# lucaspk512/vrdone

Hardware: AMD Instinct MI355X
Metric: subject-object pairs/sec forward (2048 pairs x 256 frames x 512-d) (higher is better)
Workload: dtype f16x3: f32 products as 3 scaled-f16 MFMA products (~22-bit), f32 accumulate; reference-grade: distance to a float64 run of the reference <= 1.4 x the reference's own float32 error (tests/golden/mask_vrd_f64.npz)

## Files before the change

vrdone_amd/csrc/vrd_rowops.hip:

```cpp
#include "vrd_common.h"
#include "vrd_box_feats.h"
#include <cmath>

namespace {

constexpr float LN_EPS = 1e-5f;

__device__ __forceinline__ float4 ld4(const float* p) { return *reinterpret_cast<const float4*>(p); }
__device__ __forceinline__ void st4(float* p, float4 v) { *reinterpret_cast<float4*>(p) = v; }
__device__ __forceinline__ float4 f4add(float4 a, float4 b) { return make_float4(a.x + b.x, a.y + b.y, a.z + b.z, a.w + b.w); }

__global__ __launch_bounds__(256) void bct_to_btc_kernel(const float* __restrict__ src, int C_total, int T, int c0,
                                                         int count, float* __restrict__ dst, int64_t ld_dst, int pair, int T_src,
                                                         const int32_t* __restrict__ src_batch, unsigned* rflag) {
    __shared__ float tile[64][65];
    vrd::RangeTrack rt;
    const int b = blockIdx.z, ct = blockIdx.y * 64, tt = blockIdx.x * 64;
    const int tx = threadIdx.x & 63, ty = threadIdx.x >> 6;
    const float* s = src + ((int64_t)(src_batch ? src_batch[b] : b) * C_total + c0) * T_src;
    for (int c = ty; c < 64; c += 4)
        tile[c][tx] = (ct + c < count && tt + tx < T) ? s[(int64_t)(ct + c) * T_src + tt + tx] : 0.f;
    __syncthreads();
    for (int t = ty; t < 64; t += 4)
        if (tt + t < T && ct + tx < count) {
            float* row = dst + ((int64_t)b * T + tt + t) * ld_dst;
            if (pair) vrd::store_pair1(row, ct + tx, count, tile[tx][t], pair, &rt);
            else row[ct + tx] = tile[tx][t];
        }
    rt.report(rflag, vrd::RANGE_INPUT);
}

__global__ __launch_bounds__(256) void bct_to_btc_vec_kernel(const float* __restrict__ src, int C_total, int T, int c0,
                                                             int count, float* __restrict__ dst, int64_t ld_dst, int pair, int T_src,
                                                             const int32_t* __restrict__ src_batch, unsigned* rflag) {
    __shared__ float tile[64][65];
    vrd::RangeTrack rt;
    const int b = blockIdx.z, ct = blockIdx.y * 64, tt = blockIdx.x * 64;
    const float* s = src + ((int64_t)(src_batch ? src_batch[b] : b) * C_total + c0) * T_src;
    {
        const int tx = threadIdx.x & 15, ty = threadIdx.x >> 4;
#pragma unroll
        for (int c = ty; c < 64; c += 16) {
            float4 v = make_float4(0.f, 0.f, 0.f, 0.f);
            if (ct + c < count && tt + 4 * tx < T) v = ld4(s + (int64_t)(ct + c) * T_src + tt + 4 * tx);
            tile[c][4 * tx] = v.x, tile[c][4 * tx + 1] = v.y, tile[c][4 * tx + 2] = v.z, tile[c][4 * tx + 3] = v.w;
        }
    }
    __syncthreads();
#pragma unroll
    for (int k = 0; k < 4; ++k) {
        const int id = threadIdx.x + 256 * k;
        const int cg = id & 15, t = id >> 4;
        if (tt + t >= T || ct + 4 * cg >= count) continue;
        const float4 v = make_float4(tile[4 * cg][t], tile[4 * cg + 1][t], tile[4 * cg + 2][t], tile[4 * cg + 3][t]);
        float* row = dst + ((int64_t)b * T + tt + t) * ld_dst;
        if (pair) vrd::store_pair4(row, ct + 4 * cg, count, v, pair, &rt);
        else st4(row + ct + 4 * cg, v);
    }
    rt.report(rflag, vrd::RANGE_INPUT);
}

__global__ __launch_bounds__(256) void btc_to_bct_kernel(const float* __restrict__ src, int64_t ld_src, int C, int T,
                                                         float* __restrict__ dst) {
    __shared__ float tile[64][65];
    const int b = blockIdx.z, ct = blockIdx.y * 64, tt = blockIdx.x * 64;
    const int tx = threadIdx.x & 63, ty = threadIdx.x >> 6;
    for (int t = ty; t < 64; t += 4)
        tile[t][tx] = (tt + t < T && ct + tx < C) ? src[((int64_t)b * T + tt + t) * ld_src + ct + tx] : 0.f;
    __syncthreads();
    for (int c = ty; c < 64; c += 4)
        if (ct + c < C && tt + tx < T) dst[((int64_t)b * C + ct + c) * T + tt + tx] = tile[tx][c];
}

__device__ __forceinline__ void pack_segment(const float* src, bool live, int lane, int width, float* dst, int pair,
                                             vrd::RangeTrack* rt = nullptr) {
    for (int c = lane; c < width; c += 64) {
        const float v = live ? src[c] : 0.f;
        if (pair) vrd::store_pair1(dst, c, width, v, pair, rt);
        else dst[c] = v;
    }
}

__global__ __launch_bounds__(256) void pack_pairs_kernel(vrd_pack_args a, unsigned* rflag) {
    vrd::RangeTrack rt;
    const int lane = threadIdx.x & 63;
    const int64_t row = (int64_t)blockIdx.x * 4 + __builtin_amdgcn_readfirstlane(threadIdx.x >> 6);
    if (row >= (int64_t)a.P * a.T) return;
    const int p = (int)(row / a.T), t = (int)(row - (int64_t)p * a.T);
    const bool live = t < a.lens[p];
    const float* src = a.src[p] + (int64_t)t * a.C_in;
    const int64_t half = (int64_t)a.P * a.T;
    int c0 = 0;
    pack_segment(src + c0, live, lane, a.V, a.vis + row * a.V, a.pair_wide, &rt);              c0 += a.V;
    pack_segment(src + c0, live, lane, a.V, a.vis + (half + row) * a.V, a.pair_wide, &rt);     c0 += a.V;
    if (a.Cc) {
        pack_segment(src + c0, live, lane, a.Cc, a.clip + row * a.Cc, a.pair_wide, &rt);          c0 += a.Cc;
        pack_segment(src + c0, live, lane, a.Cc, a.clip + (half + row) * a.Cc, a.pair_wide, &rt); c0 += a.Cc;
    }
    pack_segment(src + c0, live, lane, a.S, a.so_box + row * a.S, 0);                     c0 += a.S;
    pack_segment(src + c0, live, lane, a.E, a.ent + row * a.E, 0);                        c0 += a.E;
    pack_segment(src + c0, live, lane, a.E, a.ent + (half + row) * a.E, 0);
    rt.report(rflag, vrd::RANGE_INPUT);
}

using vrd::Box4;
using vrd::load_box;
using vrd::entity_feats;

__global__ __launch_bounds__(256) void gather_pairs_kernel(vrd_gather_args a, unsigned* rflag) {
    vrd::RangeTrack rt;
    const int lane = threadIdx.x & 63;
    const int64_t row = (int64_t)blockIdx.x * 4 + __builtin_amdgcn_readfirstlane(threadIdx.x >> 6);
    if (row >= (int64_t)a.P * a.T) return;
    const int p = (int)(row / a.T), t = (int)(row - (int64_t)p * a.T);
    const int n = a.lens[p];
    const bool live = t < n;
    const int64_t rs = a.s_row[p] + (int64_t)t * a.stride, ro = a.o_row[p] + (int64_t)t * a.stride;
    const int64_t half = (int64_t)a.P * a.T;
    if (a.out_vis) {
        pack_segment(a.vis + (live ? rs : 0) * a.V, live, lane, a.V, a.out_vis + row * a.V, a.pair_wide, &rt);
        pack_segment(a.vis + (live ? ro : 0) * a.V, live, lane, a.V, a.out_vis + (half + row) * a.V, a.pair_wide, &rt);
        if (a.Cc) {
            pack_segment(a.clip + (live ? rs : 0) * a.Cc, live, lane, a.Cc, a.out_clip + row * a.Cc, a.pair_wide, &rt);
            pack_segment(a.clip + (live ? ro : 0) * a.Cc, live, lane, a.Cc, a.out_clip + (half + row) * a.Cc, a.pair_wide, &rt);
        }
        rt.report(rflag, vrd::RANGE_INPUT);
    }
    float* const so = a.out_so_box + row * 5;
    float* const es = a.out_ent + row * 8;
    float* const eo = a.out_ent + (half + row) * 8;
    if (!live) {
        if (lane < 5) so[lane] = 0.f;
        if (lane < 8) es[lane] = 0.f, eo[lane] = 0.f;
        return;
    }
    if (lane == 0) {
        float f[5];
        vrd::so_box_feats(load_box(a.boxes, rs), load_box(a.boxes, ro), f);
#pragma unroll
        for (int i = 0; i < 5; ++i) so[i] = f[i];
    } else if (lane == 1 || lane == 2) {
        float f[8];
        const float w = a.seq_wh ? a.seq_wh[2 * (int64_t)p] : a.w, h = a.seq_wh ? a.seq_wh[2 * (int64_t)p + 1] : a.h;
        entity_feats(a.boxes, lane == 1 ? a.s_row[p] : a.o_row[p], a.stride, t, n, w, h, f);
        float* const dst = lane == 1 ? es : eo;
#pragma unroll
        for (int i = 0; i < 8; ++i) dst[i] = f[i];
    }
}

__global__ __launch_bounds__(256) void assemble_pairs_kernel(vrd_assemble_args a) {
    const int lane = threadIdx.x & 63;
    const int64_t row = (int64_t)blockIdx.x * 4 + __builtin_amdgcn_readfirstlane(threadIdx.x >> 6);
    if (row >= 2 * (int64_t)a.P * a.T) return;
    const int e = (int)(row / a.T), t = (int)(row - (int64_t)e * a.T);
    const int side = e >= a.P, p = e - side * a.P;
    const int n = a.lens[p];
    const float* src = nullptr;
    if (t < n) {
        const int64_t piece = ((int64_t)side * 2 * a.P + p) * a.L;
        const int end_len = n == a.T ? a.L : a.piece;
        if (n <= a.piece || t < a.reach) src = a.snippets + (piece + t) * a.D;
        else if (t >= n - a.reach) src = a.snippets + (piece + (int64_t)a.P * a.L + (t - (n - end_len))) * a.D;
        else src = a.streams + (a.stream_row[e] + t) * a.D;
    }
    float4* dst = reinterpret_cast<float4*>(a.out + row * a.D);
    for (int c = lane; c < a.D / 4; c += 64) dst[c] = src ? reinterpret_cast<const float4*>(src)[c] : float4{0.f, 0.f, 0.f, 0.f};
}

template <int NV, bool WIDE>
__device__ __forceinline__ int lane_chan(int i, int lane) { return WIDE ? lane * 8 + i * 4 : i * 256 + lane * 4; }

template <int NV, bool WIDE = false>
__device__ __forceinline__ void ln_rows(float4 (&v)[NV], const float* gamma, const float* beta, int lane, bool relu) {
    constexpr float inv_c = 1.0f / (256.0f * NV);
    float s = 0.f;
#pragma unroll
    for (int i = 0; i < NV; ++i) s += (v[i].x + v[i].y) + (v[i].z + v[i].w);
    const float mean = vrd::wave_sum(s) * inv_c;
    float ss = 0.f;
#pragma unroll
    for (int i = 0; i < NV; ++i) {
        v[i].x -= mean; v[i].y -= mean; v[i].z -= mean; v[i].w -= mean;
        ss += (v[i].x * v[i].x + v[i].y * v[i].y) + (v[i].z * v[i].z + v[i].w * v[i].w);
    }
    const float inv = 1.0f / sqrtf(vrd::wave_sum(ss) * inv_c + LN_EPS);
#pragma unroll
    for (int i = 0; i < NV; ++i) {
        const float4 g = ld4(gamma + lane_chan<NV, WIDE>(i, lane)), bb = ld4(beta + lane_chan<NV, WIDE>(i, lane));
        v[i].x = fmaf(v[i].x * inv, g.x, bb.x);
        v[i].y = fmaf(v[i].y * inv, g.y, bb.y);
        v[i].z = fmaf(v[i].z * inv, g.z, bb.z);
        v[i].w = fmaf(v[i].w * inv, g.w, bb.w);
        if (relu) {
            v[i].x = fmaxf(v[i].x, 0.f); v[i].y = fmaxf(v[i].y, 0.f);
            v[i].z = fmaxf(v[i].z, 0.f); v[i].w = fmaxf(v[i].w, 0.f);
        }
    }
}

template <int NV>
__global__ __launch_bounds__(256) void layernorm_kernel(const float* __restrict__ x, int64_t ldx, float* __restrict__ y,
                                                        int64_t ldy, int64_t rows, const float* __restrict__ gamma,
                                                        const float* __restrict__ beta, int relu,
                                                        const float* __restrict__ post_add, int64_t ld_add, int period,
                                                        int pair, unsigned* rflag) {
    vrd::RangeTrack rt;
    const int lane = threadIdx.x & 63;
    int64_t row = (int64_t)blockIdx.x * 4 + __builtin_amdgcn_readfirstlane(threadIdx.x >> 6);
    const int64_t stride = (int64_t)gridDim.x * 4;
    if (row >= rows) return;
    float4 v[NV], vn[NV];
#pragma unroll
    for (int i = 0; i < NV; ++i) v[i] = ld4(x + row * ldx + i * 256 + lane * 4);
    for (;;) {
        const int64_t nxt = row + stride;
        if (nxt < rows) {
#pragma unroll
            for (int i = 0; i < NV; ++i) vn[i] = ld4(x + nxt * ldx + i * 256 + lane * 4);
        }
        ln_rows<NV>(v, gamma, beta, lane, relu != 0);
        if (post_add) {
            const float* a = post_add + (row % period) * ld_add;
#pragma unroll
            for (int i = 0; i < NV; ++i) v[i] = f4add(v[i], ld4(a + i * 256 + lane * 4));
        }
#pragma unroll
        for (int i = 0; i < NV; ++i) {
            if (pair) vrd::store_pair4(y + row * ldy, i * 256 + lane * 4, 256 * NV, v[i], pair, &rt);
            else st4(y + row * ldy + i * 256 + lane * 4, v[i]);
        }
        if (nxt >= rows) break;
        row = nxt;
#pragma unroll
        for (int i = 0; i < NV; ++i) v[i] = vn[i];
    }
    rt.report(rflag, vrd::RANGE_LAYERNORM);
}

constexpr int CL_MAXK = 32;
template <int NV>
__global__ __launch_bounds__(256) void conv_ln_kernel(vrd_conv_ln_args p, unsigned* rflag) {
    vrd::RangeTrack rt;
    constexpr int N = 256 * NV;
    constexpr bool WIDE = NV == 2;
    extern __shared__ __attribute__((aligned(16))) float cl_lds[];
    const int K = p.Cin * p.taps;
    for (int idx = threadIdx.x; idx < N * K; idx += 256) {
        const int n = idx / K, rem = idx - n * K, ci = rem / p.taps, tap = rem - ci * p.taps;
        cl_lds[(tap * p.Cin + ci) * N + n] = p.w[idx];
    }
    for (int n = threadIdx.x; n < N; n += 256) cl_lds[K * N + n] = p.bias ? p.bias[n] : 0.f;
    __syncthreads();
    const int lane = threadIdx.x & 63;
    constexpr int RG = 4;
    int64_t grp = (int64_t)blockIdx.x * 4 + __builtin_amdgcn_readfirstlane(threadIdx.x >> 6);
    const int64_t stride = (int64_t)gridDim.x * 4;
    const int half = p.taps / 2;
    const int lrow = lane / p.Cin, lci = lane - lrow * p.Cin;
    auto load_in = [&](int64_t g) {
        const int64_t r = g * RG - half + lrow;
        float val = 0.f;
        if (lrow < RG + 2 * half && r >= 0 && r < p.rows) val = p.x[r * p.ldx + lci];
        return val;
    };
    float xin = grp * RG < p.rows ? load_in(grp) : 0.f;
    for (; grp * RG < p.rows; grp += stride) {
        const int64_t row0 = grp * RG;
        const float xcur = xin;
        if ((grp + stride) * RG < p.rows) xin = load_in(grp + stride);
        float4 v[RG][NV];
        int t[RG];
#pragma unroll
        for (int j = 0; j < RG; ++j) {
            t[j] = (int)((row0 + j) % p.T);
#pragma unroll
            for (int i = 0; i < NV; ++i) v[j][i] = *reinterpret_cast<const float4*>(cl_lds + K * N + lane_chan<NV, WIDE>(i, lane));
        }
        for (int tap = 0; tap < p.taps; ++tap) {
            for (int ci = 0; ci < p.Cin; ++ci) {
                const float* wk = cl_lds + (tap * p.Cin + ci) * N;
                float4 w[NV];
#pragma unroll
                for (int i = 0; i < NV; ++i) w[i] = *reinterpret_cast<const float4*>(wk + lane_chan<NV, WIDE>(i, lane));
#pragma unroll
                for (int j = 0; j < RG; ++j) {
                    const int tt = t[j] + tap - half;
                    const bool ok = tt >= 0 && tt < p.T && row0 + j < p.rows;
                    const float xl = __builtin_bit_cast(float, __builtin_amdgcn_readlane(__builtin_bit_cast(int, xcur), (j + tap) * p.Cin + ci));
                    const float xv = ok ? xl : 0.f;
#pragma unroll
                    for (int i = 0; i < NV; ++i) {
                        v[j][i].x = fmaf(w[i].x, xv, v[j][i].x); v[j][i].y = fmaf(w[i].y, xv, v[j][i].y);
                        v[j][i].z = fmaf(w[i].z, xv, v[j][i].z); v[j][i].w = fmaf(w[i].w, xv, v[j][i].w);
                    }
                }
            }
        }
#pragma unroll
        for (int j = 0; j < RG; ++j) {
            const int64_t row = row0 + j;
            if (row >= p.rows) break;
            if (p.row_mask) {
                const float mk = (float)vrd::uniform_load(p.row_mask + row);
#pragma unroll
                for (int i = 0; i < NV; ++i) v[j][i].x *= mk, v[j][i].y *= mk, v[j][i].z *= mk, v[j][i].w *= mk;
            }
            if (p.gamma) {
                ln_rows<NV, WIDE>(v[j], p.gamma, p.beta, lane, p.relu != 0);
            } else if (p.relu) {
#pragma unroll
                for (int i = 0; i < NV; ++i) {
                    v[j][i].x = fmaxf(v[j][i].x, 0.f); v[j][i].y = fmaxf(v[j][i].y, 0.f);
                    v[j][i].z = fmaxf(v[j][i].z, 0.f); v[j][i].w = fmaxf(v[j][i].w, 0.f);
                }
            }
            float* yr = p.y + row * p.ldy;
            if (WIDE && p.out_pair) {
                vrd::store_pair8(yr, lane * 8, v[j][0], v[j][NV - 1], p.out_pair, &rt);
            } else {
#pragma unroll
                for (int i = 0; i < NV; ++i) {
                    const int c = lane_chan<NV, WIDE>(i, lane);
                    if (p.out_pair) vrd::store_pair4(yr, c, N, v[j][i], p.out_pair, &rt);
                    else st4(yr + c, v[j][i]);
                }
            }
        }
    }
    rt.report(rflag, vrd::RANGE_LAYERNORM);
}

constexpr int DW_RW = 16;

template <int NV, int KS, int GIN>
__global__ __launch_bounds__(256) void dwconv_ln_kernel(vrd_dwconv_ln_args p, int Tout_u, int strips_per_seq, int strips_per_wave, int rw, unsigned* rflag,
                                                        vrd::SegTable sg) {
    vrd::RangeTrack rt;
    constexpr int C = 256 * NV, NT = GIN * KS, SETF = (NT + 3) * C;
    constexpr bool WIDE = NV == 2 && GIN == 1;
    extern __shared__ __attribute__((aligned(16))) float dw_lds[];
    const int lane = threadIdx.x & 63, wave = __builtin_amdgcn_readfirstlane(threadIdx.x >> 6);
    for (int o = 0; o < p.n_out; ++o) {
        float* const ls = dw_lds + o * SETF;
        if (p.packed[o]) {
            for (int idx = threadIdx.x * 4; idx < SETF; idx += 1024) st4(ls + idx, ld4(p.packed[o] + idx));
            continue;
        }
        for (int idx = threadIdx.x; idx < C * NT; idx += 256) ls[(idx % NT) * C + idx / NT] = p.w[o][idx];
        for (int c = threadIdx.x; c < C; c += 256) {
            ls[NT * C + c] = p.bias[o] ? p.bias[o][c] : 0.f;
            ls[(NT + 1) * C + c] = p.gamma[o] ? p.gamma[o][c] : 1.f;
            ls[(NT + 2) * C + c] = p.gamma[o] ? p.beta[o][c] : 0.f;
        }
    }
    const float* const pre = dw_lds + p.n_out * SETF;
    if (p.pre_gamma)
        for (int c = threadIdx.x; c < C; c += 256) {
            dw_lds[p.n_out * SETF + c] = p.pre_gamma[c];
            dw_lds[p.n_out * SETF + C + c] = p.pre_beta[c];
        }
    __syncthreads();
    const int nwg = gridDim.x, bid = blockIdx.x;
    const int xcd = bid & 7, qq = nwg >> 3, rem = nwg & 7;
    const int lid = (xcd < rem ? xcd * (qq + 1) : rem * (qq + 1) + (xcd - rem) * qq) + (bid >> 3);
    for (int si = 0; si < strips_per_wave; ++si) {
    const int64_t ws = ((int64_t)lid * 4 + wave) * strips_per_wave + si;
    int Tin, Tout, to0;
    int64_t xrow0, urow0, orow0;
    if (sg.count) {
        int g, b, strip;
        if (!vrd::seg_find(sg, ws, g, b, strip)) break;
        Tin = sg.T[g], Tout = Tin / p.stride, to0 = strip * rw;
        xrow0 = sg.row[g] + (int64_t)b * Tin;
        urow0 = sg.row[g] / 2 + (int64_t)b * (Tin / 2);
        orow0 = sg.row[g] / p.stride + (int64_t)b * Tout;
    } else {
        const int b = (int)(ws / strips_per_seq);
        if (b >= p.B) break;
        Tin = p.Tin, Tout = Tout_u, to0 = (int)(ws - (int64_t)b * strips_per_seq) * rw;
        xrow0 = (int64_t)b * Tin, urow0 = (int64_t)b * (Tin / 2), orow0 = (int64_t)b * Tout;
    }
    const int to1 = min(to0 + rw, Tout);

    struct Row {
        float4 v[NV][GIN];
    };
    auto load_row = [&](int ti) {
        Row r;
        const bool ok = ti >= 0 && ti < Tin;
#pragma unroll
        for (int i = 0; i < NV; ++i)
#pragma unroll
            for (int g = 0; g < GIN; ++g) {
                float4 v = make_float4(0.f, 0.f, 0.f, 0.f);
                if (ok) {
                    const int64_t coff = (int64_t)GIN * lane_chan<NV, WIDE>(i, lane) + 4 * g;
                    v = ld4(p.x + (xrow0 + ti) * p.ldx + coff);
                    if (p.x_up) v = f4add(v, ld4(p.x_up + (urow0 + (ti >> 1)) * p.ldx_up + coff));
                }
                r.v[i][g] = v;
            }
        if (GIN == 1 && p.pre_gamma && ok) {
            float4 t[NV];
#pragma unroll
            for (int i = 0; i < NV; ++i) t[i] = r.v[i][0];
            ln_rows<NV, WIDE>(t, pre, pre + C, lane, false);
#pragma unroll
            for (int i = 0; i < NV; ++i) r.v[i][0] = t[i];
        }
        return r;
    };
    if (p.mask_out) {
        const int64_t r0 = orow0 + to0;
        const bool mine = lane < to1 - to0 && p.mask_out[r0 + lane] != 0;
        if (!__any(mine)) {
#pragma unroll
            for (int o = 0; o < 3; ++o) {
                if (o >= p.n_out) break;
                const float* const lb = dw_lds + o * SETF + (NT + 2) * C;
                float4 val[NV];
#pragma unroll
                for (int i = 0; i < NV; ++i) {
                    val[i] = *reinterpret_cast<const float4*>(lb + lane_chan<NV, WIDE>(i, lane));
                    if (p.relu[o]) {
                        val[i].x = fmaxf(val[i].x, 0.f); val[i].y = fmaxf(val[i].y, 0.f);
                        val[i].z = fmaxf(val[i].z, 0.f); val[i].w = fmaxf(val[i].w, 0.f);
                    }
                }
                for (int to = to0; to < to1; ++to) {
                    const int64_t row = orow0 + to;
                    if (WIDE && p.out_pair[o]) {
                        vrd::store_pair8(p.y[o] + row * p.ldy[o], lane * 8, val[0], val[NV - 1], p.out_pair[o], &rt);
                    } else {
#pragma unroll
                        for (int i = 0; i < NV; ++i) {
                            const int c = lane_chan<NV, WIDE>(i, lane);
                            if (p.out_pair[o]) vrd::store_pair4(p.y[o] + row * p.ldy[o], c, 256 * NV, val[i], p.out_pair[o], &rt);
                            else st4(p.y[o] + row * p.ldy[o] + c, val[i]);
                        }
                    }
                }
            }
            continue;
        }
    }
    Row win[KS];
#pragma unroll
    for (int k = 0; k < KS; ++k) win[k] = load_row(p.stride * to0 + k - KS / 2);
    for (int to = to0; to < to1; ++to) {
        Row nxt[2];
        const int tn = p.stride * (to + 1) - KS / 2;
        const bool more = to + 1 < to1;
        if (KS == 1) {
            if (more) nxt[0] = load_row(tn);
        } else if (p.stride == 1) {
            if (more) nxt[0] = load_row(tn + 2);
        } else {
            if (more) {
                nxt[0] = load_row(tn + 1);
                nxt[1] = load_row(tn + 2);
            }
        }
        const int64_t row = orow0 + to;
        const float mk = p.mask_out ? (float)p.mask_out[row] : 1.f;
#pragma unroll
        for (int o = 0; o < 3; ++o) {
            if (o >= p.n_out) break;
            const float* const ls = dw_lds + o * SETF;
            float4 acc[NV];
#pragma unroll
            for (int i = 0; i < NV; ++i) {
                const int c = lane_chan<NV, WIDE>(i, lane);
                float4 r = *reinterpret_cast<const float4*>(ls + NT * C + c);
#pragma unroll
                for (int k = 0; k < KS; ++k) {
                    if (GIN == 1) {
                        const float4 w = *reinterpret_cast<const float4*>(ls + k * C + c);
                        const float4 v = win[k].v[i][0];
                        r.x += w.x * v.x; r.y += w.y * v.y; r.z += w.z * v.z; r.w += w.w * v.w;
                    } else {
                        const float4 w0 = *reinterpret_cast<const float4*>(ls + (0 * KS + k) * C + c);
                        const float4 w1 = *reinterpret_cast<const float4*>(ls + (1 * KS + k) * C + c);
                        const float4 v0 = win[k].v[i][0], v1 = win[k].v[i][GIN - 1];
                        r.x += w0.x * v0.x + w1.x * v0.y;
                        r.y += w0.y * v0.z + w1.y * v0.w;
                        r.z += w0.z * v1.x + w1.z * v1.y;
                        r.w += w0.w * v1.z + w1.w * v1.w;
                    }
                }
                acc[i] = make_float4(r.x * mk, r.y * mk, r.z * mk, r.w * mk);
            }
            if (p.gamma[o]) {
                ln_rows<NV, WIDE>(acc, ls + (NT + 1) * C, ls + (NT + 2) * C, lane, p.relu[o] != 0);
            } else if (p.relu[o]) {
#pragma unroll
                for (int i = 0; i < NV; ++i) {
                    acc[i].x = fmaxf(acc[i].x, 0.f); acc[i].y = fmaxf(acc[i].y, 0.f);
                    acc[i].z = fmaxf(acc[i].z, 0.f); acc[i].w = fmaxf(acc[i].w, 0.f);
                }
            }
            if (WIDE && p.out_pair[o]) {
                vrd::store_pair8(p.y[o] + row * p.ldy[o], lane * 8, acc[0], acc[NV - 1], p.out_pair[o], &rt);
            } else {
#pragma unroll
                for (int i = 0; i < NV; ++i) {
                    const int c = lane_chan<NV, WIDE>(i, lane);
                    if (p.out_pair[o]) vrd::store_pair4(p.y[o] + row * p.ldy[o], c, 256 * NV, acc[i], p.out_pair[o], &rt);
                    else st4(p.y[o] + row * p.ldy[o] + c, acc[i]);
                }
            }
        }
        if (more) {
            if (KS == 1) {
                win[0] = nxt[0];
            } else if (p.stride == 1) {
                win[0] = win[1];
                win[KS > 1 ? 1 : 0] = win[KS - 1];
                win[KS - 1] = nxt[0];
            } else {
                win[0] = win[KS - 1];
                win[KS > 1 ? 1 : 0] = nxt[0];
                win[KS - 1] = nxt[1];
            }
        }
    }
    }
    rt.report(rflag, vrd::RANGE_DWCONV_LN);
}

__global__ __launch_bounds__(256) void maxpool_mask_kernel(const float* __restrict__ x, int64_t ldx, int B, int Tin, int C,
                                                           const uint8_t* __restrict__ mask_in, float* __restrict__ y,
                                                           int64_t ldy, uint8_t* __restrict__ mask_out) {
    const int c4 = C / 4;
    const int64_t idx = (int64_t)blockIdx.x * 256 + threadIdx.x;
    const int Tout = Tin / 2;
    if (idx >= (int64_t)B * Tout * c4) return;
    const int c = (int)(idx % c4) * 4;
    const int64_t row = idx / c4;
    const int b = (int)(row / Tout), to = (int)(row - (int64_t)b * Tout);
    const float* base = x + ((int64_t)b * Tin + 2 * to) * ldx + c;
    float4 m = ld4(base);
    const float4 r = ld4(base + ldx);
    m.x = fmaxf(m.x, r.x); m.y = fmaxf(m.y, r.y); m.z = fmaxf(m.z, r.z); m.w = fmaxf(m.w, r.w);
    if (to > 0) {
        const float4 l = ld4(base - ldx);
        m.x = fmaxf(m.x, l.x); m.y = fmaxf(m.y, l.y); m.z = fmaxf(m.z, l.z); m.w = fmaxf(m.w, l.w);
    }
    const uint8_t mk = mask_in[(int64_t)b * Tin + 2 * to];
    const float f = (float)mk;
    st4(y + row * ldy + c, make_float4(m.x * f, m.y * f, m.z * f, m.w * f));
    if (c == 0 && mask_out) mask_out[row] = mk;
}

constexpr int MH_D = 256, MH_TT = 32, MH_QMAX = 16;

__global__ __launch_bounds__(256) void mask_head_kernel(const float* __restrict__ emb, int64_t ld_emb,
                                                        const float* __restrict__ feat, int64_t ld_feat,
                                                        const uint8_t* __restrict__ out_mask, int Q, int T, float fill,
                                                        float* __restrict__ seg) {
    __shared__ float fs[MH_TT][MH_D + 1];
    __shared__ float es[MH_QMAX][MH_D];
    const int b = blockIdx.y, t0 = blockIdx.x * MH_TT, tid = threadIdx.x;
    for (int i = tid; i < MH_TT * (MH_D / 4); i += 256) {
        const int r = i / (MH_D / 4), c = (i % (MH_D / 4)) * 4;
        float4 v = make_float4(0.f, 0.f, 0.f, 0.f);
        if (t0 + r < T) v = ld4(feat + ((int64_t)b * T + t0 + r) * ld_feat + c);
        fs[r][c] = v.x; fs[r][c + 1] = v.y; fs[r][c + 2] = v.z; fs[r][c + 3] = v.w;
    }
    for (int i = tid; i < Q * (MH_D / 4); i += 256) {
        const int r = i / (MH_D / 4), c = (i % (MH_D / 4)) * 4;
        st4(&es[r][c], ld4(emb + ((int64_t)b * Q + r) * ld_emb + c));
    }
    __syncthreads();
    const int tt = tid & 31, qg = tid >> 5;
    if (t0 + tt >= T) return;
    const bool on = out_mask[(int64_t)b * T + t0 + tt] != 0;
    for (int q = qg; q < Q; q += 8) {
        float s = 0.f;
#pragma unroll 8
        for (int c = 0; c < MH_D; ++c) s = fmaf(es[q][c], fs[tt][c], s);
        seg[((int64_t)b * Q + q) * T + t0 + tt] = on ? s : fill;
    }
}

inline bool aligned16(const void* ptr) { return (reinterpret_cast<uintptr_t>(ptr) & 15u) == 0; }

constexpr int RB_THREADS = 1024;
__global__ __launch_bounds__(RB_THREADS) void row_blocks_kernel(const uint8_t* __restrict__ mask, int nblocks, int seg_len, int S,
                                                                int32_t* __restrict__ order, int32_t* __restrict__ n_active) {
    __shared__ int counts[RB_THREADS];
    const int tid = threadIdx.x;
    const int per = (nblocks + RB_THREADS - 1) / RB_THREADS;
    const int b0 = min(tid * per, nblocks), b1 = min(b0 + per, nblocks);
    auto active = [&](int b) {
        const uint4* q = reinterpret_cast<const uint4*>(mask + (int64_t)b * 32);
        const uint4 lo = q[0], hi = q[1];
        return ((lo.x | lo.y | lo.z | lo.w | hi.x | hi.y | hi.z | hi.w) != 0u) ? 1 : 0;
    };
    int mine = 0;
    for (int b = b0; b < b1; ++b) mine += active(b);
    counts[tid] = mine;
    __syncthreads();
    for (int d = 1; d < RB_THREADS; d <<= 1) {
        const int v = tid >= d ? counts[tid - d] : 0;
        __syncthreads();
        counts[tid] += v;
        __syncthreads();
    }
    const int total = counts[RB_THREADS - 1];
    auto start = [&](int s) { return min(s * seg_len, nblocks); };
    auto first = [&](int s) { return (int)(((int64_t)total * start(s)) / nblocks); };
    auto pads_before = [&](int s) { return start(s) - first(s); };
    int a = counts[tid] - mine;
    int i = b0 - a;
    int sa = 0, sp = 0;
    for (int b = b0; b < b1; ++b) {
        if (active(b)) {
            while (sa + 1 < S && first(sa + 1) <= a) ++sa;
            order[start(sa) + (a - first(sa))] = b;
            ++a;
        } else {
            while (sp + 1 < S && pads_before(sp + 1) <= i) ++sp;
            order[start(sp) + (first(sp + 1) - first(sp)) + (i - pads_before(sp))] = b;
            ++i;
        }
    }
    if (tid < S) n_active[tid] = first(tid + 1) - first(tid);
}

}

extern "C" {

int vrd_bct_to_btc(const float* src, int B, int C_total, int T, int c0, int count, float* dst, int64_t ld_dst,
                   int out_pair, int T_src, const int32_t* src_batch, void* stream) {
    VRD_CHECK_ARG(src && dst, "vrd_bct_to_btc: null pointer");
    if (T_src == 0) T_src = T;
    VRD_CHECK_ARG(T_src >= T, "vrd_bct_to_btc: T_src (%d) < T (%d)", T_src, T);
    VRD_CHECK_ARG(B > 0 && T > 0 && count > 0 && c0 >= 0 && c0 + count <= C_total && ld_dst >= count,
                  "vrd_bct_to_btc: bad slab c0=%d count=%d C=%d ld=%lld", c0, count, C_total, (long long)ld_dst);
    VRD_CHECK_ARG(B <= 65535, "vrd_bct_to_btc: B too large for one launch (%d)", B);
    hipStream_t s = static_cast<hipStream_t>(stream);
    vrd::ProfScope prof(VRD_K_TRANSPOSE, s, 0.0, 8.0 * B * (double)count * T);
    dim3 grid((T + 63) / 64, (count + 63) / 64, B);
    VRD_CHECK_ARG(!out_pair || (count % 32 == 0 && ld_dst % 4 == 0 && aligned16(dst)), "vrd_bct_to_btc: pair rows need count %% 32 == 0");
    const bool vec = T % 4 == 0 && T_src % 4 == 0 && count % 4 == 0 && ld_dst % 4 == 0 && aligned16(dst) && aligned16(src);
    if (vec) hipLaunchKernelGGL(bct_to_btc_vec_kernel, grid, dim3(256), 0, s, src, C_total, T, c0, count, dst, ld_dst, out_pair, T_src, src_batch, out_pair == VRD_PAIR_F16 ? vrd::range_flag() : nullptr);
    else hipLaunchKernelGGL(bct_to_btc_kernel, grid, dim3(256), 0, s, src, C_total, T, c0, count, dst, ld_dst, out_pair, T_src, src_batch, out_pair == VRD_PAIR_F16 ? vrd::range_flag() : nullptr);
    VRD_LAUNCH_CHECK();
    return 0;
}

int vrd_pack_pairs(const vrd_pack_args* a, void* stream) {
    VRD_CHECK_ARG(a && a->src && a->lens && a->vis && a->so_box && a->ent, "vrd_pack_pairs: null pointer");
    VRD_CHECK_ARG(a->P > 0 && a->T > 0 && a->V > 0 && a->S > 0 && a->E > 0 && a->Cc >= 0, "vrd_pack_pairs: bad sizes");
    VRD_CHECK_ARG(a->C_in == 2 * a->V + 2 * a->Cc + a->S + 2 * a->E, "vrd_pack_pairs: C_in %d does not match the slab widths", a->C_in);
    VRD_CHECK_ARG(a->Cc == 0 || a->clip, "vrd_pack_pairs: clip buffer missing");
    VRD_CHECK_ARG(!a->pair_wide || (a->V % 32 == 0 && a->Cc % 32 == 0), "vrd_pack_pairs: pair rows need widths %% 32 == 0");
    hipStream_t s = static_cast<hipStream_t>(stream);
    const int64_t rows = (int64_t)a->P * a->T;
    vrd::ProfScope prof(VRD_K_TRANSPOSE, s, 0.0, 8.0 * (double)rows * a->C_in);
    hipLaunchKernelGGL(pack_pairs_kernel, dim3((unsigned)((rows + 3) / 4)), dim3(256), 0, s, *a, a->pair_wide == VRD_PAIR_F16 ? vrd::range_flag() : nullptr);
    VRD_LAUNCH_CHECK();
    return 0;
}

int vrd_gather_pairs(const vrd_gather_args* a, void* stream) {
    VRD_CHECK_ARG(a && a->vis && a->boxes && a->s_row && a->o_row && a->lens && a->out_so_box && a->out_ent,
                  "vrd_gather_pairs: null pointer");
    VRD_CHECK_ARG(a->P > 0 && a->T > 0 && a->V > 0 && a->Cc >= 0 && a->stride >= 1 && a->w > 0.f && a->h > 0.f, "vrd_gather_pairs: bad sizes");
    VRD_CHECK_ARG(a->Cc == 0 || !a->out_vis || (a->clip && a->out_clip), "vrd_gather_pairs: clip buffers missing");
    VRD_CHECK_ARG(!a->pair_wide || (a->V % 32 == 0 && a->Cc % 32 == 0), "vrd_gather_pairs: pair rows need widths %% 32 == 0");
    VRD_CHECK_ARG(aligned16(a->boxes), "vrd_gather_pairs: boxes must be 16-byte aligned");
    hipStream_t s = static_cast<hipStream_t>(stream);
    const int64_t rows = (int64_t)a->P * a->T;
    vrd::ProfScope prof(VRD_K_TRANSPOSE, s, 0.0, 8.0 * (double)rows * ((a->out_vis ? 2 * a->V + 2 * a->Cc : 0) + 21));
    hipLaunchKernelGGL(gather_pairs_kernel, dim3((unsigned)((rows + 3) / 4)), dim3(256), 0, s, *a, a->pair_wide == VRD_PAIR_F16 ? vrd::range_flag() : nullptr);
    VRD_LAUNCH_CHECK();
    return 0;
}

int vrd_assemble_pairs(const vrd_assemble_args* a, void* stream) {
    VRD_CHECK_ARG(a && a->streams && a->snippets && a->stream_row && a->lens && a->out, "vrd_assemble_pairs: null pointer");
    VRD_CHECK_ARG(a->P > 0 && a->T > 0 && a->D > 0 && a->D % 4 == 0, "vrd_assemble_pairs: bad sizes");
    VRD_CHECK_ARG(a->reach >= 0 && a->piece >= 2 * a->reach && a->piece >= 1 && a->L > a->piece && a->T >= a->L,
                  "vrd_assemble_pairs: pieces of %d frames in buffers of %d (T = %d) cannot cover a reach of %d", a->piece, a->L, a->T, a->reach);
    VRD_CHECK_ARG(aligned16(a->streams) && aligned16(a->snippets) && aligned16(a->out), "vrd_assemble_pairs: rows must be 16-byte aligned");
    hipStream_t s = static_cast<hipStream_t>(stream);
    const int64_t rows = 2 * (int64_t)a->P * a->T;
    VRD_CHECK_ARG((rows + 3) / 4 < ((int64_t)1 << 31), "vrd_assemble_pairs: grid too large");
    vrd::ProfScope prof(VRD_K_TRANSPOSE, s, 0.0, 8.0 * (double)rows * a->D);
    hipLaunchKernelGGL(assemble_pairs_kernel, dim3((unsigned)((rows + 3) / 4)), dim3(256), 0, s, *a);
    VRD_LAUNCH_CHECK();
    return 0;
}

int vrd_row_blocks(const uint8_t* mask, int64_t rows, int seg_len, int32_t* order, int32_t* n_active, void* stream) {
    VRD_CHECK_ARG(mask && order && n_active, "vrd_row_blocks: null pointer");
    VRD_CHECK_ARG(rows > 0 && rows % 32 == 0 && rows / 32 < (1 << 30), "vrd_row_blocks: rows %lld must be a positive multiple of 32", (long long)rows);
    const int nblocks = (int)(rows / 32);
    VRD_CHECK_ARG(seg_len >= 1 && (nblocks + seg_len - 1) / seg_len <= 64, "vrd_row_blocks: segment length %d gives more than 64 segments", seg_len);
    VRD_CHECK_ARG(aligned16(mask), "vrd_row_blocks: mask must be 16-byte aligned");
    hipStream_t s = static_cast<hipStream_t>(stream);
    vrd::ProfScope prof(VRD_K_TRANSPOSE, s, 0.0, (double)rows + 4.0 * nblocks);
    hipLaunchKernelGGL(row_blocks_kernel, dim3(1), dim3(RB_THREADS), 0, s, mask, nblocks, seg_len, (nblocks + seg_len - 1) / seg_len, order, n_active);
    VRD_LAUNCH_CHECK();
    return 0;
}

int vrd_btc_to_bct(const float* src, int64_t ld_src, int B, int C, int T, float* dst, void* stream) {
    VRD_CHECK_ARG(src && dst, "vrd_btc_to_bct: null pointer");
    VRD_CHECK_ARG(B > 0 && B <= 65535 && T > 0 && C > 0 && ld_src >= C, "vrd_btc_to_bct: bad shape");
    hipStream_t s = static_cast<hipStream_t>(stream);
    vrd::ProfScope prof(VRD_K_TRANSPOSE, s, 0.0, 8.0 * B * (double)C * T);
    dim3 grid((T + 63) / 64, (C + 63) / 64, B);
    hipLaunchKernelGGL(btc_to_bct_kernel, grid, dim3(256), 0, s, src, ld_src, C, T, dst);
    VRD_LAUNCH_CHECK();
    return 0;
}

int vrd_layernorm(const float* x, int64_t ldx, float* y, int64_t ldy, int64_t rows, int C, const float* gamma,
                  const float* beta, int relu, const float* post_add, int64_t ld_add, int add_period, int out_pair,
                  void* stream) {
    VRD_CHECK_ARG(x && y && gamma && beta, "vrd_layernorm: null pointer");
    VRD_CHECK_ARG(C == 256 || C == 512, "vrd_layernorm: C must be 256 or 512 (got %d)", C);
    VRD_CHECK_ARG(ldx >= C && ldy >= C && ldx % 4 == 0 && ldy % 4 == 0 && aligned16(x) && aligned16(y) &&
                      aligned16(gamma) && aligned16(beta),
                  "vrd_layernorm: rows must be 16-byte aligned");
    VRD_CHECK_ARG(!post_add || (add_period > 0 && ld_add % 4 == 0 && aligned16(post_add)), "vrd_layernorm: bad post_add");
    if (rows <= 0) return 0;
    hipStream_t s = static_cast<hipStream_t>(stream);
    vrd::ProfScope prof(VRD_K_LAYERNORM, s, 0.0, 8.0 * (double)rows * C);
    unsigned* const rflag = out_pair == VRD_PAIR_F16 ? vrd::range_flag() : nullptr;
    static const int64_t max_blocks = [] { const char* e = getenv("VRD_LN_BLOCKS"); return e ? atoll(e) : 8192; }();
    const int64_t want = (rows + 3) / 4;
    dim3 grid((unsigned)(max_blocks > 0 && want > max_blocks ? max_blocks : want));
    if (C == 256)
        hipLaunchKernelGGL(layernorm_kernel<1>, grid, dim3(256), 0, s, x, ldx, y, ldy, rows, gamma, beta, relu, post_add, ld_add, add_period, out_pair, rflag);
    else
        hipLaunchKernelGGL(layernorm_kernel<2>, grid, dim3(256), 0, s, x, ldx, y, ldy, rows, gamma, beta, relu, post_add, ld_add, add_period, out_pair, rflag);
    VRD_LAUNCH_CHECK();
    return 0;
}

int vrd_conv_ln(const vrd_conv_ln_args* a, void* stream) {
    VRD_CHECK_ARG(a && a->x && a->w && a->y, "vrd_conv_ln: null pointer");
    VRD_CHECK_ARG(a->N == 256 || a->N == 512, "vrd_conv_ln: N must be 256 or 512 (got %d)", a->N);
    VRD_CHECK_ARG((a->taps == 1 || a->taps == 3) && a->Cin > 0 && a->Cin * a->taps <= CL_MAXK && (4 + a->taps - 1) * a->Cin <= 64,
                  "vrd_conv_ln: taps in {1, 3}, taps * Cin <= %d and (3 + taps) * Cin <= 64 (got %d x %d)", CL_MAXK, a->taps, a->Cin);
    VRD_CHECK_ARG(a->rows >= 0 && a->T > 0 && a->rows % a->T == 0 && a->ldx >= a->Cin, "vrd_conv_ln: bad rows / T / ldx");
    VRD_CHECK_ARG((a->gamma == nullptr) == (a->beta == nullptr), "vrd_conv_ln: gamma and beta go together");
    VRD_CHECK_ARG(a->ldy >= a->N && a->ldy % 4 == 0 && aligned16(a->y) && aligned16(a->gamma) && aligned16(a->beta),
                  "vrd_conv_ln: output rows and LayerNorm parameters must be 16-byte aligned");
    VRD_CHECK_ARG(!a->out_pair || (a->ldy % 32 == 0 && (a->out_pair == VRD_PAIR_BF16 || a->out_pair == VRD_PAIR_F16)),
                  "vrd_conv_ln: pair output needs rows that start on a 128-byte block");
    if (a->rows == 0) return 0;
    hipStream_t s = static_cast<hipStream_t>(stream);
    const int K = a->Cin * a->taps;
    vrd::ProfScope prof(VRD_K_LAYERNORM, s, 2.0 * (double)a->rows * a->N * K, 4.0 * (double)a->rows * (a->N + a->Cin));
    unsigned* const rflag = a->out_pair == VRD_PAIR_F16 ? vrd::range_flag() : nullptr;
    const size_t lds = (size_t)(K + 1) * a->N * sizeof(float);
    const int64_t want = (a->rows + 15) / 16;
    dim3 grid((unsigned)(want > 4096 ? 4096 : want));
    if (a->N == 256) {
        if (lds > 48 * 1024)
            if (int rc = vrd::reserve_lds(reinterpret_cast<const void*>(conv_ln_kernel<1>), lds, "vrd_conv_ln")) return rc;
        hipLaunchKernelGGL(conv_ln_kernel<1>, grid, dim3(256), lds, s, *a, rflag);
    } else {
        if (lds > 48 * 1024)
            if (int rc = vrd::reserve_lds(reinterpret_cast<const void*>(conv_ln_kernel<2>), lds, "vrd_conv_ln")) return rc;
        hipLaunchKernelGGL(conv_ln_kernel<2>, grid, dim3(256), lds, s, *a, rflag);
    }
    VRD_LAUNCH_CHECK();
    return 0;
}

int vrd_dwconv_ln(const vrd_dwconv_ln_args* a, void* stream) {
    VRD_CHECK_ARG(a && a->x, "vrd_dwconv_ln: null args");
    VRD_CHECK_ARG(a->C == 256 || a->C == 512, "vrd_dwconv_ln: C must be 256 or 512 (got %d)", a->C);
    VRD_CHECK_ARG(a->ksize == 1 || a->ksize == 3, "vrd_dwconv_ln: ksize must be 1 or 3");
    VRD_CHECK_ARG(a->stride == 1 || a->stride == 2, "vrd_dwconv_ln: stride must be 1 or 2");
    VRD_CHECK_ARG(a->group_in == 1 || (a->group_in == 2 && a->C == 256 && a->ksize == 3),
                  "vrd_dwconv_ln: group_in=2 is only built for C=256, ksize=3");
    VRD_CHECK_ARG(a->segs || (a->B > 0 && a->Tin > 0 && a->Tin % a->stride == 0), "vrd_dwconv_ln: Tin %% stride != 0");
    VRD_CHECK_ARG(a->n_out >= 1 && a->n_out <= 3, "vrd_dwconv_ln: n_out must be 1..3");
    VRD_CHECK_ARG((a->pre_gamma == nullptr) == (a->pre_beta == nullptr) && (!a->pre_gamma || (a->group_in == 1 && !a->x_up)),
                  "vrd_dwconv_ln: input LayerNorm needs gamma and beta, group_in == 1 and no x_up");
    VRD_CHECK_ARG(a->ldx >= (int64_t)a->C * a->group_in && a->ldx % 4 == 0 && aligned16(a->x), "vrd_dwconv_ln: bad x layout");
    VRD_CHECK_ARG(!a->x_up || (a->Tin % 2 == 0 && a->ldx_up >= (int64_t)a->C * a->group_in && a->ldx_up % 4 == 0 && aligned16(a->x_up)), "vrd_dwconv_ln: bad x_up layout");
    for (int o = 0; o < a->n_out; ++o) {
        VRD_CHECK_ARG((a->w[o] || a->packed[o]) && a->y[o] && aligned16(a->w[o]) && aligned16(a->packed[o]) && aligned16(a->y[o]) &&
                          a->ldy[o] % 4 == 0 && a->ldy[o] >= a->C,
                      "vrd_dwconv_ln: bad output set %d", o);
        VRD_CHECK_ARG((a->gamma[o] == nullptr) == (a->beta[o] == nullptr), "vrd_dwconv_ln: gamma/beta mismatch");
    }
    vrd::SegTable sg;
    sg.count = 0;
    int64_t rows_in = (int64_t)a->B * a->Tin;
    int Tmax = a->Tin;
    if (a->segs) {
        const int even = (a->x_up || a->stride == 2) ? 2 : 1;
        VRD_CHECK_ARG(vrd::seg_table(sg, a->segs, even, 16) >= 0, "vrd_dwconv_ln: bad row groups (1..%d groups, T %% %d == 0)", VRD_MAX_SEGS, even);
        rows_in = 0, Tmax = 0;
        for (int g = 0; g < sg.count; ++g) {
            VRD_CHECK_ARG(sg.row[g] % even == 0, "vrd_dwconv_ln: a group's first row must be even with stride 2 / x_up");
            rows_in += (int64_t)sg.n[g] * sg.T[g];
            Tmax = sg.T[g] > Tmax ? sg.T[g] : Tmax;
        }
    }
    const int Tout = Tmax / a->stride;
    const int64_t rows = rows_in / a->stride;
    hipStream_t s = static_cast<hipStream_t>(stream);
    vrd::ProfScope prof(VRD_K_DWCONV_LN, s, 0.0,
                        4.0 * ((double)rows_in * a->C * a->group_in * (a->x_up ? 1.5 : 1.0) + (double)rows * a->C * a->n_out));
    const size_t lds = ((size_t)a->n_out * (a->group_in * a->ksize + 3) + (a->pre_gamma ? 2 : 0)) * a->C * sizeof(float);
    static const int rw_env = [] { const char* e = getenv("VRD_DW_RW"); return e ? atoi(e) : 0; }();
    int rw = DW_RW;
    {
        const int64_t wgs_per_cu = lds ? (int64_t)(160 * 1024 / lds) : 8;
        const int64_t resident = 256 * (wgs_per_cu < 1 ? 1 : wgs_per_cu > 4 ? 4 : wgs_per_cu) * 4;
        auto strips_at = [&](int r) -> int64_t {
            return a->segs ? vrd::seg_table(sg, a->segs, a->stride, r) : (int64_t)a->B * ((Tout + r - 1) / r);
        };
        if (strips_at(DW_RW) < 6 * resident) {
            double best = 1e30;
            for (int r = 8; r <= 32; ++r) {
                const int64_t n = strips_at(r);
                const double cost = (double)((n + resident - 1) / resident) * (r + 3);
                if (cost < best - 1e-9) best = cost, rw = r;
            }
        }
        if (rw_env >= 1 && rw_env <= 64) rw = rw_env;
    }
    const int strips = (Tout + rw - 1) / rw;
    static const int spw_env = [] { const char* e = getenv("VRD_DW_SPW"); return e ? atoi(e) : 0; }();
    const int64_t total_strips = a->segs ? vrd::seg_table(sg, a->segs, a->stride, rw) : (int64_t)a->B * strips;
    const int spw = spw_env > 0 ? spw_env : 1;
    dim3 grid((unsigned)((total_strips + 4 * spw - 1) / (4 * spw))), block(256);
    bool any_f16 = false;
    for (int o = 0; o < a->n_out; ++o) any_f16 |= a->out_pair[o] == VRD_PAIR_F16;
    unsigned* const rflag = any_f16 ? vrd::range_flag() : nullptr;
#define VRD_DW(NV, KS, GIN) hipLaunchKernelGGL((dwconv_ln_kernel<NV, KS, GIN>), grid, block, lds, s, *a, Tout, strips, spw, rw, rflag, sg)
    if (a->group_in == 2) VRD_DW(1, 3, 2);
    else if (a->C == 256 && a->ksize == 3) VRD_DW(1, 3, 1);
    else if (a->C == 256) VRD_DW(1, 1, 1);
    else if (a->ksize == 3) VRD_DW(2, 3, 1);
    else VRD_DW(2, 1, 1);
#undef VRD_DW
    VRD_LAUNCH_CHECK();
    return 0;
}

int vrd_maxpool_mask(const float* x, int64_t ldx, int B, int Tin, int C, const uint8_t* mask_in, float* y, int64_t ldy,
                     uint8_t* mask_out, void* stream) {
    VRD_CHECK_ARG(x && y && mask_in, "vrd_maxpool_mask: null pointer");
    VRD_CHECK_ARG(B > 0 && Tin > 0 && Tin % 2 == 0 && C % 4 == 0, "vrd_maxpool_mask: Tin must be even, C %% 4 == 0");
    VRD_CHECK_ARG(ldx % 4 == 0 && ldy % 4 == 0 && ldx >= C && ldy >= C && aligned16(x) && aligned16(y), "vrd_maxpool_mask: bad layout");
    hipStream_t s = static_cast<hipStream_t>(stream);
    const int64_t n = (int64_t)B * (Tin / 2) * (C / 4);
    vrd::ProfScope prof(VRD_K_POOL, s, 0.0, 4.0 * (double)B * Tin * C * 1.5);
    hipLaunchKernelGGL(maxpool_mask_kernel, dim3((unsigned)((n + 255) / 256)), dim3(256), 0, s, x, ldx, B, Tin, C, mask_in, y, ldy, mask_out);
    VRD_LAUNCH_CHECK();
    return 0;
}

int vrd_mask_head(const float* emb, int64_t ld_emb, const float* feat, int64_t ld_feat, const uint8_t* out_mask, int B,
                  int Q, int T, int Dp, float fill, float* seg, void* stream) {
    VRD_CHECK_ARG(emb && feat && out_mask && seg, "vrd_mask_head: null pointer");
    VRD_CHECK_ARG(Dp == MH_D, "vrd_mask_head: mask dim must be %d (got %d)", MH_D, Dp);
    VRD_CHECK_ARG(Q >= 1 && Q <= MH_QMAX, "vrd_mask_head: num queries must be 1..%d (got %d)", MH_QMAX, Q);
    VRD_CHECK_ARG(B > 0 && B <= 65535 && T > 0, "vrd_mask_head: bad B/T");
    VRD_CHECK_ARG(ld_emb % 4 == 0 && ld_feat % 4 == 0 && aligned16(emb) && aligned16(feat), "vrd_mask_head: bad layout");
    hipStream_t s = static_cast<hipStream_t>(stream);
    vrd::ProfScope prof(VRD_K_MASK_HEAD, s, 2.0 * B * (double)Q * T * Dp, 4.0 * B * ((double)T * Dp + (double)Q * Dp + (double)Q * T));
    hipLaunchKernelGGL(mask_head_kernel, dim3((T + MH_TT - 1) / MH_TT, B), dim3(256), 0, s, emb, ld_emb, feat, ld_feat, out_mask, Q, T, fill, seg);
    VRD_LAUNCH_CHECK();
    return 0;
}

}
```

Before: 15540.

## Split row-block compaction into parallel ballot flag pass and bitmap scatter

Row-block activity detection moves to a multi-block kernel that packs one bit per 32-row block with wave ballots into the order buffer. A single-block kernel then loads the bitmap into shared memory, counts with popcount per wave, and scatters active and inactive block indices into per-segment slots. The old kernel, where one workgroup read the whole mask, stays as a fallback for very large inputs. This adds a second launch and more complex segment-offset tracking, which could introduce ordering bugs.

Measured after the change: 15540. No clear change (-0.0%).

```diff
diff --git a/vrdone_amd/csrc/vrd_rowops.hip b/vrdone_amd/csrc/vrd_rowops.hip
--- a/vrdone_amd/csrc/vrd_rowops.hip
+++ b/vrdone_amd/csrc/vrd_rowops.hip
@@ -586,9 +586,101 @@
 
 inline bool aligned16(const void* ptr) { return (reinterpret_cast<uintptr_t>(ptr) & 15u) == 0; }
 
-constexpr int RB_THREADS = 1024;
-__global__ __launch_bounds__(RB_THREADS) void row_blocks_kernel(const uint8_t* __restrict__ mask, int nblocks, int seg_len, int S,
-                                                                int32_t* __restrict__ order, int32_t* __restrict__ n_active) {
+constexpr int RB_THREADS = 1024, RB_WAVES = RB_THREADS / 64, RB_FLAG_THREADS = 256, RB_MAX_WORDS = 15 * 1024;
+
+__global__ __launch_bounds__(RB_FLAG_THREADS) void row_block_flags_kernel(const uint8_t* __restrict__ mask, int nblocks,
+                                                                          int32_t* __restrict__ bits) {
+    const int b = blockIdx.x * RB_FLAG_THREADS + threadIdx.x, lane = threadIdx.x & 63;
+    bool on = false;
+    if (b < nblocks) {
+        const uint4* q = reinterpret_cast<const uint4*>(mask + (int64_t)b * 32);
+        const uint4 lo = q[0], hi = q[1];
+        on = (lo.x | lo.y | lo.z | lo.w | hi.x | hi.y | hi.z | hi.w) != 0u;
+    }
+    const unsigned long long wave = __ballot(on);
+    const int w = (b >> 6) * 2 + lane;
+    if (lane < 2 && w * 32 < nblocks) bits[w] = (int32_t)(uint32_t)(wave >> (32 * lane));
+}
+
+__global__ __launch_bounds__(RB_THREADS) void row_blocks_kernel(int nblocks, int seg_len, int S, int32_t* order,
+                                                                int32_t* __restrict__ n_active) {
+    extern __shared__ uint32_t rb_bits[];
+    __shared__ int wave_count[RB_WAVES];
+    __shared__ int firsts[65], pads[65];
+    auto uni = [](int v) { return __builtin_amdgcn_readfirstlane(v); };
+    const int tid = threadIdx.x, lane = tid & 63, wave = uni(tid >> 6), words = (nblocks + 31) / 32;
+    for (int w = tid; w < words; w += RB_THREADS) rb_bits[w] = (uint32_t)order[w];
+    if (tid == 0) rb_bits[words] = 0u;
+    __syncthreads();
+    const int chunk = (((nblocks + RB_WAVES - 1) / RB_WAVES + 63) / 64) * 64;
+    const int c0 = min(wave * chunk, nblocks), c1 = min(c0 + chunk, nblocks);
+    int cnt = 0;
+    for (int w = (c0 >> 5) + lane, we = c0 < c1 ? (c1 + 31) >> 5 : 0; w < we; w += 64) cnt += __popc(rb_bits[w]);
+    for (int d = 32; d; d >>= 1) cnt += __shfl_xor(cnt, d, 64);
+    if (lane == 0) wave_count[wave] = cnt;
+    __syncthreads();
+    int a0 = 0, total = 0;
+    for (int v = 0; v < RB_WAVES; ++v) {
+        const int c = uni(wave_count[v]);
+        a0 += v < wave ? c : 0;
+        total += c;
+    }
+    if (tid <= S) {
+        const int start = min(tid * seg_len, nblocks);
+        const int first = (int)(((int64_t)total * start) / nblocks);
+        firsts[tid] = first;
+        pads[tid] = start - first;
+    }
+    __syncthreads();
+    if (tid < S) n_active[tid] = firsts[tid + 1] - firsts[tid];
+    auto seg_of = [&](const int* key, int v) {
+        int lo = 0, hi = S - 1;
+        while (lo < hi) {
+            const int mid = (lo + hi + 1) >> 1;
+            if (uni(key[mid]) <= v) lo = mid; else hi = mid - 1;
+        }
+        return lo;
+    };
+    constexpr int NONE = 0x7fffffff;
+    int i0 = c0 - a0;
+    int sa = seg_of(firsts, a0), sp = seg_of(pads, i0);
+    int next_a = sa + 1 < S ? uni(firsts[sa + 1]) : NONE, next_i = sp + 1 < S ? uni(pads[sp + 1]) : NONE;
+    int off_a = uni(pads[sa]), off_i = uni(firsts[sp + 1]);
+    const int k = lane & 31;
+    const uint32_t below = (1u << k) - 1u;
+    const bool upper = lane >= 32;
+    for (int base = c0; base < c1; base += 64) {
+        const uint32_t lo = (uint32_t)uni((int)rb_bits[base >> 5]), hi = (uint32_t)uni((int)rb_bits[(base >> 5) + 1]);
+        const uint32_t word = upper ? hi : lo;
+        const int b = base + lane;
+        const int a = a0 + (upper ? __popc(lo) : 0) + __popc(word & below);
+        const bool on = (word >> k) & 1u;
+        const int r = on ? a : b - a;
+        int off = on ? off_a : off_i;
+        if (b < c1 && r >= (on ? next_a : next_i)) {
+            const int* const key = on ? firsts : pads;
+            int s = (on ? sa : sp) + 1;
+            while (s + 1 < S && key[s + 1] <= r) ++s;
+            off = on ? pads[s] : firsts[s + 1];
+        }
+        if (b < c1) order[r + off] = b;
+        a0 += __popc(lo) + __popc(hi);
+        i0 = min(base + 64, c1) - a0;
+        while (a0 >= next_a) {
+            ++sa;
+            next_a = sa + 1 < S ? uni(firsts[sa + 1]) : NONE;
+            off_a = uni(pads[sa]);
+        }
+        while (i0 >= next_i) {
+            ++sp;
+            next_i = sp + 1 < S ? uni(pads[sp + 1]) : NONE;
+            off_i = uni(firsts[sp + 1]);
+        }
+    }
+}
+
+__global__ __launch_bounds__(RB_THREADS) void row_blocks_serial_kernel(const uint8_t* __restrict__ mask, int nblocks, int seg_len, int S,
+                                                                       int32_t* __restrict__ order, int32_t* __restrict__ n_active) {
     __shared__ int counts[RB_THREADS];
     const int tid = threadIdx.x;
     const int per = (nblocks + RB_THREADS - 1) / RB_THREADS;
@@ -704,7 +796,14 @@
     VRD_CHECK_ARG(aligned16(mask), "vrd_row_blocks: mask must be 16-byte aligned");
     hipStream_t s = static_cast<hipStream_t>(stream);
     vrd::ProfScope prof(VRD_K_TRANSPOSE, s, 0.0, (double)rows + 4.0 * nblocks);
-    hipLaunchKernelGGL(row_blocks_kernel, dim3(1), dim3(RB_THREADS), 0, s, mask, nblocks, seg_len, (nblocks + seg_len - 1) / seg_len, order, n_active);
+    const int S = (nblocks + seg_len - 1) / seg_len, words = (nblocks + 31) / 32;
+    if (words <= RB_MAX_WORDS) {
+        hipLaunchKernelGGL(row_block_flags_kernel, dim3((unsigned)((nblocks + RB_FLAG_THREADS - 1) / RB_FLAG_THREADS)), dim3(RB_FLAG_THREADS), 0, s, mask, nblocks, order);
+        VRD_LAUNCH_CHECK();
+        hipLaunchKernelGGL(row_blocks_kernel, dim3(1), dim3(RB_THREADS), (words + 1) * sizeof(uint32_t), s, nblocks, seg_len, S, order, n_active);
+    } else {
+        hipLaunchKernelGGL(row_blocks_serial_kernel, dim3(1), dim3(RB_THREADS), 0, s, mask, nblocks, seg_len, S, order, n_active);
+    }
     VRD_LAUNCH_CHECK();
     return 0;
 }
```
